# inferrna/Core

Hardware: AMD Instinct MI355X
Metric: Mrays/s (primary+shadow), 1M-tri scene (higher is better)
Workload: dtype f32

## Files before the change

core_amd/csrc/yk_device.hip:

```cpp
#include <hip/hip_runtime.h>

#include <algorithm>
#include <atomic>
#include <climits>
#include <chrono>
#include <cmath>
#include <cstdio>
#include <cstdlib>
#include <cstring>
#include <mutex>
#include <type_traits>
#include <stdexcept>
#include <string>
#include <thread>
#include <vector>

#include "../../include/yk_api.h"
#include "../../include/yk_test_hooks.h"
#include "../../include/yk_test_hooks_light.h"
#include "../../include/yk_test_hooks_camera.h"
#include "../../include/yk_test_hooks_film.h"
#include "../../include/yk_test_hooks_depth.h"
#include "photon_map.h"
#include "scene.h"
// ... 788 lines not shown
  std::conditional_t<CLOSEST, unsigned long long, unsigned> keys[YK_SMALL_LANE_LEAF ? 1 : 64];
  float s_tmin[(CLOSEST || UNI) ? 64 : 1];
  unsigned ray_n0[64];
  unsigned res_slot[CLOSEST ? 1 : 128];
  float4 cand[CLOSEST ? 64 : 1];
  uint2 stack[R * 64];
};
__host__ __device__ __forceinline__ unsigned small_rec_word(unsigned nn) { return (nn * 6u + 3u) & ~3u; }
__device__ __forceinline__ void small_scene_copy(const DScene& S, uint32_t* dst, int W) {
  const unsigned nthr = 64u * (unsigned)W;
  const unsigned n4 = S.nnodes * 4u, n6 = S.nnodes * 6u;
  for (unsigned i = threadIdx.x; i < n6; i += nthr) {
    const unsigned node = i < n4 ? i >> 2 : (i - n4) >> 1, w = i < n4 ? i & 3u : 4u + ((i - n4) & 1u);
    dst[i] = S.pk[node * kPkWords + w];
  }
  float* t = reinterpret_cast<float*>(dst + small_rec_word(S.nnodes));
  const unsigned nt = S.ntris * 12u, nl = S.nlref * 12u;
  for (unsigned i = threadIdx.x; i < nt + nl; i += nthr) {
    const bool own = i < nt;
    const unsigned j = own ? i : i - nt, rec = j / 12u, w = j - rec * 12u, c = w & 3u;
    const float* src = own ? S.tris : S.ltris;
    t[i] = c < 3u ? src[rec * kTriWords + (w >> 2) * 3u + c] : 0.f;
  }
}
size_t small_scene_bytes(size_t nn, size_t ntris, size_t nlref) {
  return 4 * (((6 * nn + 3) & ~(size_t)3) + 12 * (ntris + nlref));
}

constexpr unsigned kTmaxInf = 0xFFC00000u;
__device__ __forceinline__ float shadow_w(float tmax) {
  return tmax < 0.f ? __uint_as_float(kTmaxInf) : (tmax != tmax ? __uint_as_float(0x7FC00000u) : fabsf(tmax));
}
__device__ __forceinline__ yk_ray unpack_shadow(float4 dw, float4 o) {
  yk_ray r;
  r.from[0] = o.x;
  r.from[1] = o.y;
  r.from[2] = o.z;
  r.dir[0] = dw.x;
  r.dir[1] = dw.y;
  r.dir[2] = dw.z;
  const bool inf = __float_as_uint(dw.w) == kTmaxInf, mis = !inf && (__float_as_uint(dw.w) >> 31) != 0u;
  r.tmin = mis ? YK_MIN_RAYDIST : o.w;
  r.tmax = inf ? -1.f : (mis ? -dw.w : dw.w);
  return r;
}

struct RaySrc {
  const yk_ray* rays;
  const float4* sdir;
  const float4* sorg;
  unsigned omask, kshift, kstride;
};

template <bool CLOSEST, int NSEG, bool TS = false, bool BIG = false, bool UNI = false, int W = 1, bool SPLIT = false>
__device__ __forceinline__ void trace_body(DScene S, RaySrc src, const unsigned* __restrict__ idx,
                                           RayCount rc, yk_hit* __restrict__ hits, uint8_t* __restrict__ occl,
                                           unsigned long long* __restrict__ work, unsigned long long* __restrict__ ctr,
                                           uint2* __restrict__ ovf, int ovf_depth, int refill_min,
                                           float* __restrict__ tsf = nullptr, int ts_depth = 0) {
  using KeyT = std::conditional_t<CLOSEST, unsigned long long, unsigned>;
  constexpr int R = W > 1 ? YK_SMALL_RING : (CLOSEST ? kStackLdsC : kStackLds);
  unsigned* otab;
  uint2* lds;
  float* s_tmin;
  unsigned* res_slot;
  unsigned* ray_n0;
  KeyT* keys;
  float4* cand;
  const char* nbase;
  const char* nbase2 = nullptr;
  const float *tb, *lb;
  unsigned wv = 0;
  int lane;
  if constexpr (W == 1) {
    __shared__ unsigned a_otab[64];
    __shared__ uint2 a_lds[R * 64];
    __shared__ float a_tmin[(CLOSEST || UNI) ? 64 : 1];
    __shared__ unsigned a_res[(!CLOSEST && !TS) ? 128 : 1];
    __shared__ unsigned a_n0[64];
    __shared__ KeyT a_keys[64];
    __shared__ float4 a_cand[CLOSEST ? 64 : 1];
    otab = a_otab;
    lds = a_lds;
    s_tmin = a_tmin;
    res_slot = a_res;
    ray_n0 = a_n0;
    keys = a_keys;
    cand = a_cand;
    nbase = reinterpret_cast<const char*>(S.pk);
    tb = S.tris;
    lb = S.ltris;
    lane = threadIdx.x;
  } else {
    __shared__ WaveLds<CLOSEST, UNI, R> s_w[W];
    wv = (unsigned)__builtin_amdgcn_readfirstlane((int)threadIdx.x) >> 6;
    WaveLds<CLOSEST, UNI, R>& L = s_w[wv];
    otab = L.otab;
    lds = L.stack;
    s_tmin = L.s_tmin;
    res_slot = L.res_slot;
    ray_n0 = L.ray_n0;
    keys = L.keys;
    cand = L.cand;
    uint32_t* dst = reinterpret_cast<uint32_t*>(yk_dyn_lds);
    small_scene_copy(S, dst, W);
    __syncthreads();
    nbase = reinterpret_cast<const char*>(dst);
    nbase2 = reinterpret_cast<const char*>(dst + S.nnodes * 4u);
    tb = reinterpret_cast<const float*>(dst + small_rec_word(S.nnodes));
    lb = tb + S.ntris * 12u;
    lane = threadIdx.x & 63u;
  }
  const unsigned gw = blockIdx.x * (unsigned)W + wv;
  unsigned npend = 0;
  const long long n = __builtin_amdgcn_readfirstlane((int)rc.get());
  if (gw == 0 && lane == 0 && n > 0) atomicAdd(&ctr[3], (unsigned long long)n);
  if ((long long)gw * 64 >= n + 63) return;
  const LaneStackT<R> stk{lds, ovf, (unsigned)ovf_depth, gw};
  int rid = -1;
  bool exhausted = false;
  Trav st;
  unsigned nnodes = 0, ntris = 0, nerr = 0;
#ifndef YK_POOL_CHUNKS
#define YK_POOL_CHUNKS 16
#endif
#ifndef YK_POOL_CHUNK_MAX
#define YK_POOL_CHUNK_MAX 512
#endif
  const unsigned kPoolChunk = (unsigned)__builtin_amdgcn_readfirstlane((int)max(
      64u, min(min((unsigned)YK_POOL_CHUNK_MAX, S.chunk_max),
               (unsigned)(n / ((long long)gridDim.x * W * YK_POOL_CHUNKS)) & ~63u)));
  unsigned xcc;
  asm volatile("s_getreg_b32 %0, hwreg(HW_REG_XCC_ID, 0, 4)" : "=s"(xcc));
  constexpr unsigned kAll = (1u << NSEG) - 1u;
  const unsigned seg_len = (unsigned)((n + NSEG - 1) / NSEG);
  unsigned pool_next = 0, pool_end = 0;
  unsigned seg_done = 0;

  unsigned iters = 0;
#ifdef YK_TRAV_STATS
  unsigned long long s_it = 0, s_act = 0, s_dmax = 0, s_lmax = 0, s_refill = 0;
  unsigned long long c_ref = 0, c_desc = 0, c_leaf = 0, c_pop = 0, c_t0 = clock64();
#endif
  for (;;) {
    const unsigned long long want = __ballot(rid < 0 && !exhausted);
    const unsigned long long act = __ballot(rid >= 0);
    if (want != 0ull && (act == 0ull || __popcll(want) >= refill_min)) {
#ifdef YK_TRAV_STATS
      s_refill++;
#endif
      const unsigned cnt = (unsigned)__popcll(want);
      const unsigned avail = pool_end - pool_next;
      unsigned cb = 0, ce = 0;
      if (avail < cnt && seg_done != kAll) {
#pragma unroll 1
        for (unsigned k = 0; k < (unsigned)NSEG; ++k) {
          const unsigned sgi = (xcc + k) % (unsigned)NSEG;
          if (seg_done & (1u << sgi)) continue;
          const unsigned long long s0 = (unsigned long long)sgi * seg_len;
          const unsigned long long s1 = min(s0 + seg_len, (unsigned long long)n);
          unsigned long long base = 0;
          if (lane == 0) base = atomicAdd(work + 16 * sgi, (unsigned long long)kPoolChunk);
          base = s0 + shfl_u64(base, 0);
          if (base < s1) {
            cb = (unsigned)__builtin_amdgcn_readfirstlane((int)(unsigned)base);
            ce = (unsigned)__builtin_amdgcn_readfirstlane((int)(unsigned)min(base + kPoolChunk, s1));
            break;
          }
          seg_done |= 1u << sgi;
        }
      }
      if (rid < 0 && !exhausted) {
        const unsigned rank = __builtin_amdgcn_mbcnt_hi((unsigned)(want >> 32),
                                                         __builtin_amdgcn_mbcnt_lo((unsigned)want, 0u));
        long long q = -1;
        if (rank < avail) q = pool_next + rank;
        else if (rank - avail < ce - cb) q = cb + (rank - avail);
        if (q < 0) {
          exhausted = (seg_done == kAll);
        } else {
          int r;
          yk_ray ray;
          if constexpr (!SPLIT) {
            r = idx ? (int)idx[q] : (int)q;
            ray = src.rays[r];
          } else {
            const unsigned e = idx ? idx[q] : (unsigned)q, oi = e & src.omask;
            r = (int)((e >> src.kshift) * src.kstride + oi);
            ray = unpack_shadow(src.sdir[r], src.sorg[oi]);
          }
          if (TS) st.ts_max = ts_depth;
          if (trav_begin<CLOSEST, TS, UNI>(S, st, ray)) {
            rid = r;
            ray_n0[lane_fresh()] = nnodes;
            if (CLOSEST || UNI) s_tmin[lane_fresh()] = st.tmin;
          } else if (CLOSEST) {
#ifndef YK_NO_CLOSEST_RESULTS
            const unsigned m1 = vconst<0xFFFFFFFFu>(), z = vconst<0u>();
            hits[r] = yk_hit{(int)m1, __uint_as_float(z), __uint_as_float(z), __uint_as_float(z)};
#endif
          } else {
            occl[r] = 0;
            if (TS) {
              tsf[3 * (size_t)r] = 1.f;
              tsf[3 * (size_t)r + 1] = 1.f;
              tsf[3 * (size_t)r + 2] = 1.f;
            }
          }
        }
      }
      if (avail < cnt) {
        const unsigned take = min(cnt - avail, ce - cb);
        pool_next = cb + take;
        pool_end = ce;
      } else {
        pool_next += cnt;
      }
      pool_next = (unsigned)__builtin_amdgcn_readfirstlane((int)pool_next);
      pool_end = (unsigned)__builtin_amdgcn_readfirstlane((int)pool_end);
    }
#ifdef YK_TRAV_STATS
    {
      const unsigned long long t = clock64();
      c_ref += t - c_t0;
      c_t0 = t;
    }
#endif
    if (__ballot(rid >= 0) == 0ull) {
      if (__ballot(!exhausted) == 0ull) break;
      continue;
    }
    bool runaway = false;
    if ((++iters & 31u) == 0u) runaway = rid >= 0 && nnodes - ray_n0[lane_fresh()] > S.nnodes + 2u;
#ifdef YK_TRAV_STATS
    const unsigned n_before = nnodes, t_before = ntris;
    s_it++;
    s_act += (unsigned long long)__popcll(__ballot(rid >= 0));
#endif
    if constexpr (!TS) {
      const bool act = rid >= 0;
      bool live = false;
      uint32_t w0 = 0, nref = 0;
      bool paused = false;
      if (act) live = trav_descend<CLOSEST, (W > 1)>(S, nbase, nbase2, st, stk, nnodes, w0, nref, paused);
#ifdef YK_TRAV_STATS
      asm volatile("s_waitcnt vmcnt(0) lgkmcnt(0)" ::: "memory");
      {
        const unsigned long long t = clock64();
        c_desc += t - c_t0;
        c_t0 = t;
      }
#endif
      bool occ = false;
      if constexpr (W > 1 && YK_SMALL_LANE_LEAF)
        lane_leaves<CLOSEST, UNI>(tb, lb, st, (live && !paused) ? nref : 0u, w0, cand, s_tmin, ntris, occ);
      else
        coop_leaves<CLOSEST, BIG, UNI, W>(S, tb, lb, st, (live && !paused) ? nref : 0u, w0, keys, cand, otab, s_tmin,
                                           ntris, occ);
#ifdef YK_TRAV_STATS
      asm volatile("s_waitcnt vmcnt(0) lgkmcnt(0)" ::: "memory");
      {
        const unsigned long long t = clock64();
        c_leaf += t - c_t0;
        c_t0 = t;
      }
#endif
      bool fin = false;
      int fin_rid = 0;
      if (act) {
        bool done = !live || occ || (!paused && trav_next<CLOSEST>(S, st, stk));
        if (runaway) {
          st.sp = kSpError;
          done = true;
        }
        const bool err = st.sp == kSpError;
        if (err) nerr++;
        if (done) {
          if (CLOSEST) {
            yk_hit h{-1, 0.f, 0.f, 0.f};
            if (st.Z < st.dist && !err) {
              const float4 c = cand[lane_fresh()];
              unsigned p = __float_as_uint(c.w);
// ... 93 lines not shown
  if (!CLOSEST && !TS && npend) {
    wave_lds_sync<W>();
    const int l = lane_fresh();
    if ((unsigned)l < npend) {
      const unsigned e = res_slot[l];
#ifndef YK_NO_SHADOW_RESULTS
      occl[e >> 1] = (uint8_t)(e & 1u);
#endif
    }
  }
  unsigned long long a = nnodes, b = ntris;
#pragma unroll
  for (int off = 32; off > 0; off >>= 1) {
    a += shfl_u64(a, lane ^ off);
    b += shfl_u64(b, lane ^ off);
  }
  if (lane == 0 && (a | b)) {
    atomicAdd(&ctr[0], a);
    atomicAdd(&ctr[1], b);
  }
  if (nerr) atomicAdd(&ctr[2], (unsigned long long)nerr);
}

#ifndef YK_SHADOW_SEGS
#define YK_SHADOW_SEGS 8
#endif
#ifndef YK_CLOSEST_WAVES
#define YK_CLOSEST_WAVES 7
#endif
#ifndef YK_SHADOW_WAVES
#define YK_SHADOW_WAVES 7
#endif

__global__ void __launch_bounds__(64) __attribute__((amdgpu_waves_per_eu(YK_CLOSEST_WAVES)))
k_trace_closest(DScene S, RaySrc src, const unsigned* __restrict__ idx, RayCount n,
                yk_hit* __restrict__ hits, uint8_t* __restrict__ occl, unsigned long long* __restrict__ work,
                unsigned long long* __restrict__ ctr, uint2* __restrict__ ovf, int ovf_depth, int refill_min) {
  trace_body<true, 8>(S, src, idx, n, hits, occl, work, ctr, ovf, ovf_depth, refill_min);
}
__global__ void __launch_bounds__(64) __attribute__((amdgpu_waves_per_eu(YK_SHADOW_WAVES)))
k_trace_shadow(DScene S, RaySrc src, const unsigned* __restrict__ idx, RayCount n,
               yk_hit* __restrict__ hits, uint8_t* __restrict__ occl, unsigned long long* __restrict__ work,
               unsigned long long* __restrict__ ctr, uint2* __restrict__ ovf, int ovf_depth, int refill_min) {
  trace_body<false, YK_SHADOW_SEGS>(S, src, idx, n, hits, occl, work, ctr, ovf, ovf_depth, refill_min);
}
__global__ void __launch_bounds__(64) __attribute__((amdgpu_waves_per_eu(YK_SHADOW_WAVES)))
k_trace_shadow_split(DScene S, RaySrc src, const unsigned* __restrict__ idx, RayCount n,
                     yk_hit* __restrict__ hits, uint8_t* __restrict__ occl, unsigned long long* __restrict__ work,
                     unsigned long long* __restrict__ ctr, uint2* __restrict__ ovf, int ovf_depth, int refill_min) {
  trace_body<false, YK_SHADOW_SEGS, false, false, false, 1, true>(S, src, idx, n, hits, occl, work, ctr, ovf,
                                                                   ovf_depth, refill_min);
}
__global__ void __launch_bounds__(64) __attribute__((amdgpu_waves_per_eu(YK_CLOSEST_WAVES)))
k_trace_closest_big(DScene S, RaySrc src, const unsigned* __restrict__ idx, RayCount n,
                    yk_hit* __restrict__ hits, uint8_t* __restrict__ occl, unsigned long long* __restrict__ work,
                    unsigned long long* __restrict__ ctr, uint2* __restrict__ ovf, int ovf_depth, int refill_min) {
  trace_body<true, 8, false, true>(S, src, idx, n, hits, occl, work, ctr, ovf, ovf_depth, refill_min);
}
__global__ void __launch_bounds__(64) __attribute__((amdgpu_waves_per_eu(YK_SHADOW_WAVES)))
k_trace_shadow_big(DScene S, RaySrc src, const unsigned* __restrict__ idx, RayCount n,
                   yk_hit* __restrict__ hits, uint8_t* __restrict__ occl, unsigned long long* __restrict__ work,
                   unsigned long long* __restrict__ ctr, uint2* __restrict__ ovf, int ovf_depth, int refill_min) {
  trace_body<false, 1, false, true>(S, src, idx, n, hits, occl, work, ctr, ovf, ovf_depth, refill_min);
}
__global__ void __launch_bounds__(64) __attribute__((amdgpu_waves_per_eu(YK_SHADOW_WAVES)))
k_trace_shadow_uni(DScene S, RaySrc src, const unsigned* __restrict__ idx, RayCount n,
                   yk_hit* __restrict__ hits, uint8_t* __restrict__ occl, unsigned long long* __restrict__ work,
                   unsigned long long* __restrict__ ctr, uint2* __restrict__ ovf, int ovf_depth, int refill_min) {
  trace_body<false, 1, false, false, true>(S, src, idx, n, hits, occl, work, ctr, ovf, ovf_depth,
                                                        refill_min);
}
__global__ void __launch_bounds__(64) __attribute__((amdgpu_waves_per_eu(YK_SHADOW_WAVES)))
k_trace_shadow_big_uni(DScene S, RaySrc src, const unsigned* __restrict__ idx, RayCount n,
                       yk_hit* __restrict__ hits, uint8_t* __restrict__ occl, unsigned long long* __restrict__ work,
                       unsigned long long* __restrict__ ctr, uint2* __restrict__ ovf, int ovf_depth, int refill_min) {
  trace_body<false, 1, false, true, true>(S, src, idx, n, hits, occl, work, ctr, ovf, ovf_depth, refill_min);
}
__global__ void __launch_bounds__(64) __attribute__((amdgpu_waves_per_eu(5)))
k_trace_shadow_ts(DScene S, RaySrc src, const unsigned* __restrict__ idx, RayCount n,
                  uint8_t* __restrict__ occl, float* __restrict__ tsf, int ts_depth, unsigned long long* __restrict__ work,
                  unsigned long long* __restrict__ ctr, uint2* __restrict__ ovf, int ovf_depth, int refill_min) {
  trace_body<false, 1, true>(S, src, idx, n, nullptr, occl, work, ctr, ovf, ovf_depth, refill_min, tsf,
                                    ts_depth);
}
__global__ void __launch_bounds__(64 * YK_SMALL_W) __attribute__((amdgpu_waves_per_eu(YK_CLOSEST_WAVES)))
k_trace_closest_small(DScene S, RaySrc src, const unsigned* __restrict__ idx, RayCount n,
                      yk_hit* __restrict__ hits, uint8_t* __restrict__ occl, unsigned long long* __restrict__ work,
                      unsigned long long* __restrict__ ctr, uint2* __restrict__ ovf, int ovf_depth, int refill_min) {
  trace_body<true, 8, false, false, false, YK_SMALL_W>(S, src, idx, n, hits, occl, work, ctr, ovf, ovf_depth,
                                                       refill_min);
}
__global__ void __launch_bounds__(64 * YK_SMALL_W) __attribute__((amdgpu_waves_per_eu(YK_SHADOW_WAVES)))
k_trace_shadow_small(DScene S, RaySrc src, const unsigned* __restrict__ idx, RayCount n,
                     yk_hit* __restrict__ hits, uint8_t* __restrict__ occl, unsigned long long* __restrict__ work,
                     unsigned long long* __restrict__ ctr, uint2* __restrict__ ovf, int ovf_depth, int refill_min) {
  trace_body<false, YK_SHADOW_SEGS, false, false, false, YK_SMALL_W>(S, src, idx, n, hits, occl, work, ctr, ovf,
                                                                     ovf_depth, refill_min);
}
__global__ void __launch_bounds__(64 * YK_SMALL_W) __attribute__((amdgpu_waves_per_eu(YK_SHADOW_WAVES)))
k_trace_shadow_small_split(DScene S, RaySrc src, const unsigned* __restrict__ idx, RayCount n,
                           yk_hit* __restrict__ hits, uint8_t* __restrict__ occl, unsigned long long* __restrict__ work,
                           unsigned long long* __restrict__ ctr, uint2* __restrict__ ovf, int ovf_depth,
                           int refill_min) {
  trace_body<false, YK_SHADOW_SEGS, false, false, false, YK_SMALL_W, true>(S, src, idx, n, hits, occl, work, ctr,
                                                                           ovf, ovf_depth, refill_min);
}
__global__ void __launch_bounds__(64 * YK_SMALL_W) __attribute__((amdgpu_waves_per_eu(YK_SHADOW_WAVES)))
k_trace_shadow_uni_small(DScene S, RaySrc src, const unsigned* __restrict__ idx, RayCount n,
                         yk_hit* __restrict__ hits, uint8_t* __restrict__ occl, unsigned long long* __restrict__ work,
                         unsigned long long* __restrict__ ctr, uint2* __restrict__ ovf, int ovf_depth, int refill_min) {
  trace_body<false, 1, false, false, true, YK_SMALL_W>(S, src, idx, n, hits, occl, work, ctr, ovf, ovf_depth,
                                                       refill_min);
}



__device__ __forceinline__ SurfPt make_surface(const DScene& S, v3 from, v3 dir, const yk_hit& h) {
  SurfPt sp;
  sp.P = vadd(from, vmul(h.t, dir));
  const float4 g = S.ng[h.prim];
  sp.Ng = V3(g.x, g.y, g.z);
  sp.N = sp.Ng;
  const int mw = __float_as_int(g.w);
  sp.mat = mw & (kSmoothBit - 1);
  if (mw & kSmoothBit) {
    const float* vn = S.vn + 9 * (size_t)h.prim;
    const float b0 = S.uni ? 0.0f : 1.0f - (h.b1 + h.b2);
    sp.N = vnormalize(vadd(vadd(vmul(b0, ld3(vn)), vmul(h.b1, ld3(vn + 3))), vmul(h.b2, ld3(vn + 6))));
  }
  create_cs(sp.N, sp.NU, sp.NV);
  return sp;
}

__device__ __forceinline__ v3 face_forward(v3 Ng, v3 N, v3 I) {
  return (vdot(Ng, I) < 0.f) ? vneg(N) : N;
}

__device__ __forceinline__ float mat_fresnel(const DMat& M, v3 wo, v3 N) {
  if (!M.fresnel) return 1.f;
  const float c = fabsf(N.x * wo.x + N.y * wo.y + N.z * wo.z);
  const float t = M.ior2 + c * c;
  const float g = (t < 1.f) ? 0.f : sqrtf(t - 1.f);
  const float gc = g + c, aux = gc * c;
// ... 2348 lines not shown
  return (v >= 1 && v <= kPipes) ? v : kPipes;
}

constexpr long long kNodeBytes = 116;
const char* plan_batches(const yk_batch_plan_in& in, yk_batch_plan& out) {
  out = yk_batch_plan{};
  out.status = YK_ERR_UNSUPPORTED;
  if (in.slots > (1 << 20) || in.bounces < 0 || in.bounces > 62) return "too many shadow slots or bounces";
  const int K = std::max(1, in.slots);
  const int pipes_cfg = std::min(kPipes, std::max(1, in.pipes));
  const long long owned = std::max<long long>(0, in.owned_tiles);
  const int regions = in.merged ? in.bounces + 1 : 1;
  out.regions = regions;
  const long long region_bytes = in.split ? 34ll * K + 16 : 50ll * K;
  const long long bytes_per_sample = 400 + 2ll * K + region_bytes + (long long)(regions - 1) * (region_bytes + 32) +
                                     (in.transp_shadows ? 28ll * K : 0) + ((in.reserved & 1) ? 4 : 0);
  out.bytes_per_sample = bytes_per_sample;
  const long long target_env = in.target_samples > 0 ? in.target_samples : (32ll << 20);
  const long long target =
      std::min(target_env, std::max(1ll << 20, std::max<long long>(0, in.budget_bytes) / pipes_cfg / bytes_per_sample));
  const long long tile_samples = (long long)in.tile * in.tile * in.spp;
  if (in.tile < 1 || in.spp < 1) return "empty tile";
  const long long spec_worst = (2ll << std::max(0, std::min(in.spec_levels, 19))) - 1;
  if (in.spec && spec_worst * tile_samples * kNodeBytes > (48ll << 30))
    return "raydepth too large for the tile size / spp (node store > 48 GB)";
  const long long target_spec = in.spec ? std::min(target, (12ll << 30) / (kNodeBytes * spec_worst)) : target;
  const long long tiles_fill = in.spec ? LLONG_MAX : (owned + pipes_cfg - 1) / pipes_cfg;
  long long tiles_per_batch =
      std::max<long long>(1, std::min<long long>(INT_MAX, std::min(target_spec / tile_samples, tiles_fill)));
  auto index_fits = [&](long long mc) {
    if (mc >= (1ll << 31)) return false;
    int kshift = 0;
    while ((1ll << kshift) < mc * regions) ++kshift;
    return mc * (long long)K * regions < (1ll << 31) && kshift <= 31 && ((long long)(K - 1) << kshift) < (1ll << 32);
  };
  while (tiles_per_batch > 1 && !index_fits(tiles_per_batch * tile_samples)) tiles_per_batch /= 2;
  const long long maxc = tiles_per_batch * tile_samples;
  if (!index_fits(maxc)) return "one tile holds too many samples (tile^2 * spp * shadow slots * regions >= 2^31)";
  out.tiles_per_batch = (int)tiles_per_batch;
  out.maxc = maxc;
  out.kstride = maxc * regions;
  while ((1ll << out.kshift) < out.kstride) ++out.kshift;
  out.nbatch = (int)((owned + tiles_per_batch - 1) / tiles_per_batch);
  out.npipes = in.spec ? 1 : std::min(pipes_cfg, std::max(1, out.nbatch));
  out.status = YK_OK;
  return nullptr;
}

enum TraceVariant {
  kClosest, kShadow, kShadowSplit,
  kClosestBig, kShadowBig,
  kShadowUni, kShadowBigUni,
  kClosestSmall, kShadowSmall, kShadowSmallSplit, kShadowUniSmall,
  kTraceVariants
};
using TraceKernel = void (*)(DScene, RaySrc, const unsigned*, RayCount, yk_hit*, uint8_t*, unsigned long long*,
                             unsigned long long*, uint2*, int, int);
struct TraceInfo {
  TraceKernel kernel;
  int waves;
  bool dyn_lds;
  int ring;
};
constexpr TraceInfo kTrace[kTraceVariants] = {
    {k_trace_closest, 1, false, kStackLdsC},
    {k_trace_shadow, 1, false, kStackLds},
    {k_trace_shadow_split, 1, false, kStackLds},
    {k_trace_closest_big, 1, false, kStackLdsC},
    {k_trace_shadow_big, 1, false, kStackLds},
    {k_trace_shadow_uni, 1, false, kStackLds},
    {k_trace_shadow_big_uni, 1, false, kStackLds},
    {k_trace_closest_small, YK_SMALL_W, true, YK_SMALL_RING},
    {k_trace_shadow_small, YK_SMALL_W, true, YK_SMALL_RING},
    {k_trace_shadow_small_split, YK_SMALL_W, true, YK_SMALL_RING},
    {k_trace_shadow_uni_small, YK_SMALL_W, true, YK_SMALL_RING},
};

struct yk_device {
  int ordinal = 0;
  int cus = 0;
  int per_cu[kTraceVariants] = {};
  bool small = false;
  size_t small_bytes = 0;
  hipStream_t stream = nullptr;
  bool uploaded = false;
  const yk_scene* uploaded_scene = nullptr;
  uint64_t uploaded_gen = 0;
  uint64_t const_token = 0;
  size_t nleaf = 0;
  DBuf<float> tris;
  DBuf<float4> ng;
  DBuf<float> vn;
  DBuf<uint2> nodes;
  DBuf<uint32_t> pk;
  DBuf<float> ltris;
  DBuf<uint32_t> leaf;
  DScene S{};
  int ntris = 0, max_depth = 0, nlights = 0, sum_light_slots = 0;
  bool spec = false;
  int xl_lights = 0;
  DBuf<DMeshLight> ml_recs;
  DBuf<float> ml_f;
  DBuf<uint2> ml_nodes;
  DBuf<uint32_t> ml_leaf;
  bool diff_only = false;
  yk_abort_fn abort_fn = nullptr;
  void* abort_user = nullptr;
  bool big_leaves = false;
  bool crowded_leaves = false;
  int refill = 24;
  int refill_shadow = 24;
  int per_cu_ts = 1;
  int per_cu_lookup[2] = {1, 1};
  DBuf<float> nE, nD, nP, nrcol, nalpha, nmalpha;
  DBuf<int> nflags, nchild, noverflow;
  DBuf<yk_ray> nray;
  DBuf<unsigned> nsoffs, npsample;
  DBuf<unsigned long long> ncount, spec_words;
  bool has_bg = false;
  float bg[3] = {0.f, 0.f, 0.f};
  std::vector<DLight> lights_host;
  bool pm_ready = false;
  int pm_integrator = -1;
  yk_photon_params pm_params{};
  DBuf<uint2> dm_nodes, rm_nodes, cm_nodes;
  DBuf<float4> dm_pos, dm_dir, dm_col, rm_pos, rm_dir, rm_col, cm_pos, cm_dir, cm_col;
  DBuf<uint4> rm_pk;
  std::vector<float> dm_host, rm_host, cm_host;
// ... 345 lines not shown
        *err = "kd-tree leaf " + std::to_string(i) + " references out of range";
        return -1;
      }
      continue;
    }
    const uint64_t r = w1 >> 2;
    if (i + 1 >= nn || r <= i + 1 || r >= nn) {
      *err = "kd-tree node " + std::to_string(i) + " has a child out of order or range";
      return -1;
    }
    for (const uint64_t c : {(uint64_t)i + 1, r}) {
      if (++parents[c] > 1) {
        *err = "kd-tree node " + std::to_string(c) + " has two parents";
        return -1;
      }
      if (depth[i] >= kMaxTreeDepth) {
        *err = "kd-tree deeper than 64 levels (KD_MAX_STACK)";
        return -1;
      }
      depth[c] = (uint8_t)(depth[i] + 1);
      maxd = std::max(maxd, (int)depth[c]);
    }
  }
  for (size_t i = 1; i < nn; ++i)
    if (parents[i] != 1) {
      *err = "kd-tree node " + std::to_string(i) + " is unreachable";
      return -1;
    }
  return maxd;
}

void set_tree_bounds(yk_device* d, int depth) {
  d->max_depth = depth;
  d->S.depth_cap = (unsigned)depth + 2u;
}
int stack_depth(const yk_device* d) { return (int)d->S.depth_cap + 2 * (int)kDescTrips + 2; }

int refill_env() {
  static const int v = [] {
    const char* e = std::getenv("YK_REFILL");
    const int r = e ? std::atoi(e) : 0;
    return (r >= 1 && r <= 64) ? r : 0;
  }();
  return v;
}

inline RaySrc ray_src(const yk_ray* r) { return RaySrc{r, nullptr, nullptr, 0u, 0u, 0u}; }
inline RaySrc shadow_src(const Batch& B) {
  if (!B.split) return ray_src(reinterpret_cast<const yk_ray*>(B.s_dir));
  return RaySrc{nullptr, B.s_dir, B.s_dir + (long long)B.K * B.kstride, (1u << B.kshift) - 1u, (unsigned)B.kshift,
                (unsigned)B.kstride};
}

TraceVariant trace_variant(const yk_device* d, bool closest, bool split) {
  const bool small = d->small && !d->big_leaves;
  if (split) return small ? kShadowSmallSplit : kShadowSplit;
  if (small) return closest ? kClosestSmall : d->S.uni ? kShadowUniSmall : kShadowSmall;
  if (closest) return d->big_leaves ? kClosestBig : kClosest;
  if (d->S.uni) return d->big_leaves ? kShadowBigUni : kShadowUni;
  return d->big_leaves ? kShadowBig : kShadow;
}

void fill_trace_occupancy(yk_device* d, bool dyn_lds) {
  for (int v = 0; v < kTraceVariants; ++v) {
    const TraceInfo& t = kTrace[v];
    if (t.dyn_lds != dyn_lds) continue;
    int blocks = 0;
    HIPCHK(hipOccupancyMaxActiveBlocksPerMultiprocessor(&blocks, t.kernel, 64 * t.waves,
                                                        dyn_lds ? d->small_bytes : 0));
    d->per_cu[v] = std::max(1, blocks);
  }
  if (dyn_lds) return;
  d->per_cu[kShadowUni] = d->per_cu[kShadow];
  d->per_cu[kShadowBigUni] = d->per_cu[kShadowBig];
}

template <bool CLOSEST>
void enqueue_trace(yk_device* d, Pipe& P, RaySrc rays, const unsigned* idx, RayCount n, yk_hit* hits,
                   uint8_t* occ, unsigned long long* work, unsigned long long* acc, hipEvent_t ev0, hipEvent_t ev1) {
  const TraceVariant v = trace_variant(d, CLOSEST, !CLOSEST && rays.rays == nullptr);
  const TraceInfo& t = kTrace[v];
  const long long grid = (long long)d->cus * d->per_cu[v];
  const int ovf_depth = std::max(1, stack_depth(d) - t.ring);
  P.ovf.ensure((size_t)ovf_depth * (size_t)grid * 64 * t.waves);
  if (ev0) HIPCHK(hipEventRecord(ev0, P.stream));
  launch(t.kernel, (unsigned)grid, 64 * t.waves, t.dyn_lds ? d->small_bytes : 0, P.stream, d->S, rays, idx, n, hits,
         occ, work, acc, P.ovf.p, ovf_depth, CLOSEST ? d->refill : d->refill_shadow);
  if (ev1) HIPCHK(hipEventRecord(ev1, P.stream));
}

void enqueue_trace_ts(yk_device* d, Pipe& P, RaySrc rays, const unsigned* idx, RayCount n, uint8_t* occ,
                      float* filt, int max_depth, unsigned long long* work, unsigned long long* acc, hipEvent_t ev0,
                      hipEvent_t ev1) {
  const long long grid = (long long)d->cus * d->per_cu_ts;
  const int ovf_depth = std::max(1, stack_depth(d) - kStackLds);
  P.ovf.ensure((size_t)ovf_depth * (size_t)grid * 64);
  if (ev0) HIPCHK(hipEventRecord(ev0, P.stream));
  launch(k_trace_shadow_ts, (unsigned)grid, 64, 0, P.stream, d->S, rays, idx, n, occ, filt, max_depth, work, acc,
         P.ovf.p, ovf_depth, d->refill_shadow);
  if (ev1) HIPCHK(hipEventRecord(ev1, P.stream));
}

bool lookup_lds(const yk_device* d) { return d->rm_depth <= kLdsPStack && d->rm_nnodes < 65536; }
size_t lookup_lds_bytes(int depth) { return (size_t)std::max(1, depth) * 64 * (sizeof(float) + sizeof(unsigned short)); }

inline int ao_slots(const yk_render_params* p) {
  return (p->integrator == YK_INTEGRATOR_DIRECT && p->do_ao) ? std::max(0, p->ao_samples) : 0;
}
bool shadow_split(const yk_device* d, const yk_render_params* p) {
  const char* e = std::getenv("YK_SPLIT");
  const long long K = std::max<long long>(1, (long long)d->sum_light_slots + ao_slots(p));
  return (e ? std::atoi(e) != 0 : K >= 4) && !d->S.uni && !d->big_leaves && !p->transp_shadows;
}

void add_trace_stats(yk_stats* st, bool closest, uint64_t rays, uint64_t nodes, uint64_t tris, double ms,
                     uint64_t launches = 1) {
  if (closest) {
    st->closest_rays += rays;
    st->closest_nodes += nodes;
    st->closest_tris += tris;
    st->ms_closest += ms;
    st->closest_launches += launches;
  } else {
    st->shadow_rays += rays;
    st->shadow_nodes += nodes;
    st->shadow_tris += tris;
    st->ms_shadow += ms;
    st->shadow_launches += launches;
  }
}

template <bool CLOSEST>
void launch_trace(yk_device* d, Pipe& P, const yk_ray* rays, long long n, yk_hit* hits, uint8_t* occ, yk_stats* st,
// ... 514 lines not shown
```

core_amd/csrc/yk_render_host.inc:

```
struct PassSpec {
  int n, off;
  bool multipass;
  const uint8_t* flags;
  float* d_depth = nullptr;
};

namespace {

bool needs_photon_maps(const yk_render_params* p) {
  return p->integrator == YK_INTEGRATOR_PHOTON ||
         (p->integrator == YK_INTEGRATOR_PATH &&
          (p->caustic_type == YK_CAUSTIC_PHOTON || p->caustic_type == YK_CAUSTIC_BOTH)) ||
         (p->integrator == YK_INTEGRATOR_DIRECT && p->dl_caustics != 0);
}

int check_tiles(const yk_render_params* p) {
  const int tile = p->tile_size > 0 ? p->tile_size : 32;
  if (tile > 4096) return set_error(YK_ERR_UNSUPPORTED, "tile_size > 4096");
  const int ntiles = ((p->width + tile - 1) / tile) * ((p->height + tile - 1) / tile);
  if (ntiles >= (1 << 19)) return set_error(YK_ERR_UNSUPPORTED, "too many tiles");
  if (p->tile_order && p->tile_order_len > 0) {
    if (p->tile_order_len != ntiles)
      return set_error(YK_ERR_ARG, "tile_order must list every tile of the render area once");
    std::vector<char> seen((size_t)ntiles, 0);
// ... 98 lines not shown
        for (int yy = Y; yy < Y + H; ++yy)
          for (int xx = X; xx < X + W; ++xx) {
            const size_t px = (size_t)(yy - F.cy0) * F.w + (xx - F.cx0);
            if (!flags[px]) continue;
            L.pmap[px] = (int)nc;
            L.pix.push_back((yy << 16) | xx);
            nc += spp;
          }
      } else {
        nc += (long long)W * H * spp;
      }
      rx0 = std::min(rx0, X);
      ry0 = std::min(ry0, Y);
      rx1 = std::max(rx1, X + W);
      ry1 = std::max(ry1, Y + H);
    }
    L.base[(size_t)bi * (tpb + 1) + (tb1 - tb0)] = (int)nc;
    L.nc_of[bi] = nc;
    L.rect_of[bi] = make_int4(rx0, ry0, rx1, ry1);
  }
}

struct FilmOptions {
  bool clamp, premult;
};
inline FilmOptions film_options(const yk_render_params* p) { return FilmOptions{p->clamp_rgb != 0, p->premult_alpha != 0}; }
void launch_film_gather(hipStream_t stream, const FilmConst& F, const int* pmap, int tb0, int tb1, int4 rect,
                        long long nc, const float4* samples, const float2* sxy, const int* base, char4* pext,
                        float* d_film, FilmOptions opt = FilmOptions{false, false}, const float* depths = nullptr,
                        float* d_depth = nullptr) {
  FilmConst Fb = F;
  Fb.pmap = pmap;
  Fb.tb0 = tb0;
  Fb.tb1 = tb1;
  const int gx0 = std::max(F.cx0, rect.x + F.olo_x), gy0 = std::max(F.cy0, rect.y + F.olo_y);
  const int gx1 = std::min(F.cx1, rect.z + F.ohi_x), gy1 = std::min(F.cy1, rect.w + F.ohi_y);
  const int gw = gx1 - gx0, gh = gy1 - gy0;
  if (nc > 0 && gw > 0 && gh > 0) {
    const long long npix = nc / F.spp;
    launch(k_pixel_extent, grid_for(npix * 64), 256, 0, stream, Fb, sxy, pext, npix);
    auto* gather = opt.clamp ? (opt.premult ? k_film_gather<true, true> : k_film_gather<true, false>)
                             : (opt.premult ? k_film_gather<false, true> : k_film_gather<false, false>);
    if (samples)
      launch(gather, grid_for((long long)gw * gh), 256, 0, stream, Fb, samples, sxy, base, pext, d_film, gx0, gy0, gw,
             gh);
    if (depths)
      launch(k_depth_gather, grid_for((long long)gw * gh), 256, 0, stream, Fb, depths, sxy, base, pext, d_depth, gx0,
             gy0, gw, gh);
  }
}

struct FramePlan : TileLists {
  bool pm, cmap, ao, path, merged, split;
  FilmConst F;
  RenderConst R;
  AOConst AOC;
  PMConst PMC;
  int K;
  int bounces, nsub;
  int spec_levels;
  yk_batch_plan plan;
  int qwords_per_batch, launches_per_batch;
  long long words_per_batch;
};

const char* build_frame_plan(const yk_device* d, const yk_render_params* p, int32_t shard, int32_t nshards,
                             const PassSpec& ps, FramePlan& fp) {
  fp.pm = p->integrator == YK_INTEGRATOR_PHOTON;
  fp.path = p->integrator == YK_INTEGRATOR_PATH;
  const bool pt_cmap = fp.path && (p->caustic_type == YK_CAUSTIC_PHOTON || p->caustic_type == YK_CAUSTIC_BOTH);
  fp.cmap = needs_photon_maps(p) && !fp.pm;
  fp.ao = p->integrator == YK_INTEGRATOR_DIRECT && p->do_ao != 0;
  FilmConst& F = fp.F;
  F = make_film(p);
  F.shard = shard;
  F.nshards = nshards;
  F.spp = ps.n;
  F.d1 = (float)(1.0 / (double)(float)ps.n);
  F.rank_of = nullptr;
  const int spp = F.spp;
  owned_tiles(F, p->tile_order, p->tile_order_len, fp);
  RenderConst& R = fp.R;
  R = RenderConst{};
  R.spp = spp;
  R.nsub = fp.path ? std::max(1, p->path_samples) : 1;
  R.pm_fg = (fp.pm && p->photon.final_gather && !p->photon.show_map) ? 1 : 0;
  R.pm_showmap = (fp.pm && p->photon.show_map) ? 1 : 0;
  if (R.pm_fg) R.nsub = std::max(1, p->photon.fg_samples);
  fp.PMC = needs_photon_maps(p) ? pm_const(d, p->photon) : PMConst{};
  R.bounces = p->bounces;
  R.integrator = p->integrator;
  R.transp_bg = p->transp_background;
  R.nlights = d->nlights;
  R.has_bg = d->has_bg ? 1 : 0;
  for (int k = 0; k < 3; ++k) R.bg[k] = d->bg[k];
  R.d1 = F.d1;
  R.spec = d->spec ? 1 : 0;
  R.trace_caustics =
      (fp.path && (p->caustic_type == YK_CAUSTIC_PATH || p->caustic_type == YK_CAUSTIC_BOTH)) ? 1 : 0;
  R.rdepth = p->raydepth;
  R.level = 0;
  R.multipass = ps.multipass ? 1 : 0;
  R.pass_off = ps.off;
  R.ps = (R.spec || R.multipass) ? 1 : 0;
  fp.K = std::max(1, d->sum_light_slots + ao_slots(p));
  fp.AOC = AOConst{};
  if (fp.ao) {
    fp.AOC.n = p->ao_samples;
    fp.AOC.k0 = d->sum_light_slots;
    fp.AOC.dist = p->ao_distance;
    for (int k = 0; k < 3; ++k) fp.AOC.col[k] = p->ao_color[k];
  }
  fp.spec_levels = d->spec ? std::max(0, std::min(p->raydepth, 19)) : 0;
  const char* merge_env = std::getenv("YK_MERGE");
  fp.merged = !(merge_env && std::atoi(merge_env) == 0) && fp.path && !d->spec && !pt_cmap && !p->transp_shadows &&
              p->path_samples <= 1 && p->bounces >= 1;
  R.merged = fp.merged ? 1 : 0;
  static const long long batch_gb_env = [] {
    const char* e = std::getenv("YK_BATCH_GB");
    const long long v = e ? std::atoll(e) : 0;
    return (v > 0 && v <= 240) ? v : 0ll;
  }();
  fp.split = shadow_split(d, p);
  yk_batch_plan_in pin{};
  pin.slots = fp.K;
  pin.bounces = fp.merged ? p->bounces : 0;
  pin.merged = fp.merged ? 1 : 0;
  pin.split = fp.split ? 1 : 0;
  pin.transp_shadows = p->transp_shadows ? 1 : 0;
  pin.spec = d->spec ? 1 : 0;
  pin.final_gather = R.pm_fg;
  pin.spec_levels = fp.spec_levels;
  pin.tile = F.tile;
  pin.spp = spp;
  pin.pipes = pipes_env();
  pin.reserved = p->z_channel ? 1 : 0;
  pin.owned_tiles = (long long)fp.owned.size();
  const char* target_env = std::getenv("YK_BATCH_SAMPLES");
  pin.target_samples = target_env ? std::atoll(target_env) : 0;
  pin.budget_bytes = (batch_gb_env ? batch_gb_env : (fp.merged ? 192ll : 64ll)) << 30;
  if (const char* why = plan_batches(pin, fp.plan)) return why;
  fp.bounces = fp.path ? R.bounces : (R.pm_fg ? p->photon.fg_bounces + 1 : 0);
  fp.nsub = (fp.path || R.pm_fg) ? R.nsub : 1;
  fp.qwords_per_batch = fp.nsub * (fp.bounces + 1);
  fp.launches_per_batch = 2 + 2 * fp.nsub * fp.bounces + (R.pm_fg ? fp.nsub * fp.bounces : 0);
  fp.words_per_batch = 2ll * fp.qwords_per_batch + 128ll * fp.launches_per_batch;

  build_tile_lists(F, fp.plan.nbatch, fp.plan.tiles_per_batch, spp, ps.flags, fp);
  return nullptr;
}

void upload_frame_plan(yk_device* d, FramePlan& fp) {
  auto up = [](auto& dev, const auto& host, size_t at_least) {
    dev.ensure(std::max(at_least, host.size()));
    if (!host.empty())
      HIPCHK(hipMemcpy(dev.p, host.data(), host.size() * sizeof(host[0]), hipMemcpyHostToDevice));
  };
  up(d->tiles_dev, fp.tiles, 0);
  up(d->base_dev, fp.base, 0);
  if (!fp.pmap.empty()) {
    up(d->pix_dev, fp.pix, 1);
    up(d->pmap_dev, fp.pmap, 0);
  }
  if (!fp.rank_of.empty()) {
    up(d->rank_dev, fp.rank_of, 0);
    fp.F.rank_of = d->rank_dev.p;
  }
}

void bind_pipes(yk_device* d, const yk_render_params* p, const FramePlan& fp, Batch* Bp) {
  const yk_batch_plan& pl = fp.plan;
  for (int pi = 0; pi < pl.npipes; ++pi) {
    Pipe& P = d->pipe[pi];
    const int nb_here = (pl.nbatch - pi + pl.npipes - 1) / pl.npipes;
    P.words.ensure((size_t)(2 * kAccWords + (d->spec ? 0 : fp.words_per_batch * nb_here)));
    HIPCHK(hipMemsetAsync(P.words.p, 0, P.words.n * sizeof(unsigned long long), P.stream));
// ... 9 lines not shown

NodeStore bind_node_store(yk_device* d, const FramePlan& fp) {
  if (!d->spec) return NodeStore{};
  const long long cap = fp.plan.maxc * ((2ll << fp.spec_levels) - 1);
  d->nE.ensure(3 * cap);
  d->nD.ensure(3 * cap);
  d->nP.ensure(3 * cap);
  d->nrcol.ensure(6 * cap);
  d->nalpha.ensure(fp.plan.maxc);
  d->nflags.ensure(cap);
  d->nchild.ensure(2 * cap);
  d->nray.ensure(cap);
  d->nsoffs.ensure(cap);
  d->npsample.ensure(cap);
  d->ncount.ensure(1);
  d->noverflow.ensure(1);
  d->nmalpha.ensure(cap);
  d->spec_words.ensure((size_t)fp.words_per_batch);
  HIPCHK(hipMemsetAsync(d->noverflow.p, 0, sizeof(int), d->pipe[0].stream));
  return NodeStore{d->nE.p,   d->nD.p,     d->nP.p,       d->nflags.p, d->nchild.p,    d->nrcol.p,    d->nalpha.p,
                   d->nray.p, d->nsoffs.p, d->npsample.p, d->ncount.p, (long long)cap, d->noverflow.p, d->nmalpha.p};
}

struct Timed {
  int pipe;
  size_t ev;
  bool closest;
};

bool cam_can_die(const yk_device* d) { return d->cam_host.kind == YK_CAMERA_ANGULAR && d->cam_host.circular != 0; }

struct BatchCtx {
  yk_device* d;
  const yk_render_params* p;
  const FramePlan* fp;
  const PassSpec* ps;
  float* d_film;
  NodeStore NS;
  std::vector<Timed>* timed;
  size_t* evn;
  int pi;
  Pipe* P;
  Batch B;
  unsigned long long* bw;
  int launch;
  unsigned long long* live = nullptr;
  float* zs = nullptr;
  DepthConst DC{};
};

unsigned long long* qw(const BatchCtx& c, int isub, int depth) { return c.bw + isub * (c.fp->bounces + 1) + depth; }
unsigned long long* next_work(BatchCtx& c) { return c.bw + 2ll * c.fp->qwords_per_batch + 128ll * c.launch++; }

void trace(BatchCtx& c, bool closest, RaySrc rays, const unsigned* idx, RayCount n, yk_hit* hits, uint8_t* occ) {
  Pipe& P = *c.P;
  unsigned long long* work = next_work(c);
  const hipEvent_t e0 = P.event(c.evn[c.pi]), e1 = P.event(c.evn[c.pi] + 1);
  c.timed->push_back(Timed{c.pi, c.evn[c.pi], closest});
  c.evn[c.pi] += 2;
  if (closest) enqueue_trace<true>(c.d, P, rays, idx, n, hits, occ, work, P.words.p, e0, e1);
  else if (c.B.ts)
    enqueue_trace_ts(c.d, P, rays, idx, n, occ, c.B.s_filt, c.p->shadow_depth, work, P.words.p + kAccWords, e0, e1);
  else enqueue_trace<false>(c.d, P, rays, idx, n, hits, occ, work, P.words.p + kAccWords, e0, e1);
}
void trace_shadow_slots(BatchCtx& c, const Batch& Bc, RayCount n) {
  trace(c, false, shadow_src(Bc), Bc.s_idx, n, nullptr, Bc.s_occl);
}

void enqueue_photon_mapping(BatchCtx& c, const Batch& Bc, const RenderConst& Rc, long long n) {
  yk_device* d = c.d;
  Pipe& P = *c.P;
  const PMConst& PMC = c.fp->PMC;
  const int fg_bounces = c.p->photon.fg_bounces;
  if (PMC.show_map || !PMC.final_gather) launch(k_pm_post, grid_for(n, 64), 64, 0, P.stream, d->S, Bc, PMC, n);
  for (int isub = 0; isub < (Rc.pm_fg ? c.fp->nsub : 0); ++isub) {
    launch(d->diff_only ? k_fg_start<true> : k_fg_start<false>, grid_for(n, YK_APPEND_BLOCK), YK_APPEND_BLOCK, 0,
           P.stream, d->S, Bc, Rc, n, isub, P.fgl.p, qw(c, isub, 0));
    int qin = 1;
    for (int it = 0; it <= fg_bounces; ++it) {
      const unsigned long long* in_w = qw(c, isub, it);
      unsigned long long* out_w = qw(c, isub, it + 1);
      trace(c, true, ray_src(Bc.q_rays[qin]), nullptr, RayCount{in_w, 32, 0}, Bc.q_hits[qin], nullptr);
      unsigned long long* lk_w = qw(c, isub, it) + c.fp->qwords_per_batch;
      launch(d->diff_only ? k_fg_hit<true> : k_fg_hit<false>, grid_for(n, YK_APPEND_BLOCK), YK_APPEND_BLOCK, 0,
             P.stream, d->S, Bc, Rc, PMC, in_w, it, isub, qin, P.fgl.p, P.fglen.p, out_w, P.lkq.p, lk_w);
      if (it < fg_bounces) trace_shadow_slots(c, Bc, RayCount{out_w, 0, 0});
      const bool lds = lookup_lds(d);
      launch(lds ? k_pm_lookup<true> : k_pm_lookup<false>, (unsigned)((long long)d->cus * d->per_cu_lookup[lds]), 64,
             lds ? lookup_lds_bytes(d->rm_depth) : 0, P.stream, PMC.rmap, PMC.lookup_rad, d->rm_depth, P.lkq.p, lk_w,
             P.fgl.p, next_work(c));
      launch(k_fg_resolve, grid_for(n), 256, 0, P.stream, Bc, Rc, in_w, qin, P.fgl.p);
      qin ^= 1;
    }
  }
  launch(k_pm_finish, grid_for(n, 64), 64, 0, P.stream, d->S, Bc, Rc, PMC, n);
}

void enqueue_post_direct(BatchCtx& c, const Batch& Bc, const RenderConst& Rc, long long n) {
  const FramePlan& fp = *c.fp;
  hipStream_t s = c.P->stream;
  if (fp.pm) enqueue_photon_mapping(c, Bc, Rc, n);
  if (fp.cmap && fp.PMC.cmap.n != 0)
    launch(k_pt_caustic, grid_for(n, 64), 64, 0, s, c.d->S, Bc, fp.PMC, n);
  if (fp.ao) launch(k_resolve_ao, grid_for(n), 256, 0, s, c.d->S, Bc, Rc, fp.AOC, n);
}

void enqueue_entries(BatchCtx& c, const Batch& Bc, const RenderConst& Rc, long long n, long long node_base) {
  yk_device* d = c.d;
  const FramePlan& fp = *c.fp;
  hipStream_t s = c.P->stream;
  const bool merged = fp.merged;
  const bool post_direct_after_bounces = d->spec;
  if (d->spec) {
    HIPCHK(hipMemsetAsync(d->spec_words.p, 0, d->spec_words.n * sizeof(unsigned long long), s));
    c.launch = 0;
  }
  if (c.live && node_base == 0) trace(c, true, ray_src(Bc.p_rays), Bc.s_idx, RayCount{c.live, 0, 0}, Bc.p_hits, nullptr);
  else trace(c, true, ray_src(Bc.p_rays), nullptr, RayCount{nullptr, 0, n}, Bc.p_hits, nullptr);
  if (c.zs && node_base == 0) launch(k_depth_samples, grid_for(n), 256, 0, s, Bc.p_rays, Bc.p_hits, c.zs, c.DC, n);
  launch(shade_primary_fn(d->diff_only, d->xl_lights, fp.ao), grid_for(n, YK_PRIMARY_BLOCK), YK_PRIMARY_BLOCK, 0, s,
         d->S, Bc, Rc, n, qw(c, 0, 0), fp.AOC);
  if (!merged) {
    trace_shadow_slots(c, Bc, RayCount{qw(c, 0, 0), 0, 0});
    launch(k_resolve_primary, grid_for(n), 256, 0, s, Bc, Rc, n);
  }
  if (!post_direct_after_bounces) enqueue_post_direct(c, Bc, Rc, n);
  const int bblock = bounce_block(d->diff_only);
  for (int isub = 0; isub < (fp.path ? fp.nsub : 0); ++isub) {
    if (isub > 0)
      launch(d->diff_only ? k_path_start<true> : k_path_start<false>, grid_for(n, YK_BOUNCE_BLOCK), YK_BOUNCE_BLOCK, 0,
             s, d->S, Bc, Rc, n, isub, qw(c, isub, 0));
    int qin = 1;
    for (int depth = 1; depth <= fp.bounces; ++depth) {
      const unsigned long long* in_w = qw(c, isub, depth - 1);
      unsigned long long* out_w = qw(c, isub, depth);
      trace(c, true, ray_src(Bc.q_rays[qin]), nullptr, RayCount{in_w, 32, 0}, Bc.q_hits[qin], nullptr);
      Batch Bd = Bc;
      if (merged) {
        Bd = merged_region(Bc, depth);
        Bd.mq_words = qw(c, 0, 0);
      }
      launch(shade_bounce_fn(d->diff_only, d->xl_lights), grid_for(n, bblock), bblock, 0, s, d->S, Bd, Rc, in_w, depth,
             isub, qin, out_w);
      if (!merged) {
        trace_shadow_slots(c, Bc, RayCount{out_w, 0, 0});
        launch(k_resolve_bounce, grid_for(n), 256, 0, s, Bc, Rc, in_w, depth, qin);
      }
      qin ^= 1;
    }
  }
  if (post_direct_after_bounces) enqueue_post_direct(c, Bc, Rc, n);
  if (d->spec) {
    launch(k_finish_spec, grid_for(n), 256, 0, s, Bc, Rc, c.NS, node_base, n);
    launch(k_spawn, grid_for(n), 256, 0, s, d->S, Bc, Rc, c.NS, node_base, n);
  } else if (merged) {
    trace_shadow_slots(c, Bc, RayCount{qw(c, 0, 0), 0, 0, fp.plan.regions});
    launch(k_resolve_merged, grid_for(n), 256, 0, s, Bc, Rc, n, fp.bounces);
  } else {
    launch(k_finish, grid_for(n), 256, 0, s, Bc, Rc, n);
  }
}

int enqueue_spec_generations(BatchCtx& c, long long nc) {
  const FramePlan& fp = *c.fp;
  const NodeStore& NS = c.NS;
  hipStream_t s = c.P->stream;
  const long long maxc = fp.plan.maxc;
  const unsigned long long start = (unsigned long long)nc;
  HIPCHK(hipMemcpyAsync(NS.count, &start, sizeof start, hipMemcpyHostToDevice, s));
  enqueue_entries(c, c.B, fp.R, nc, 0);
  long long g0 = 0, g1 = nc;
// ... 456 lines not shown
```

Before: 3504.

## Hand out camera rays to waves in contiguous 64-ray groups

Result: faster. 3593 (median of 6 runs) (+2.5%).

```diff
diff --git a/core_amd/csrc/yk_device.hip b/core_amd/csrc/yk_device.hip
--- a/core_amd/csrc/yk_device.hip
+++ b/core_amd/csrc/yk_device.hip
@@ -864,12 +864,14 @@
   unsigned omask, kshift, kstride;
 };
 
-template <bool CLOSEST, int NSEG, bool TS = false, bool BIG = false, bool UNI = false, int W = 1, bool SPLIT = false>
+template <bool CLOSEST, int NSEG, bool TS = false, bool BIG = false, bool UNI = false, int W = 1, bool SPLIT = false,
+          bool GROUP = false>
 __device__ __forceinline__ void trace_body(DScene S, RaySrc src, const unsigned* __restrict__ idx,
                                            RayCount rc, yk_hit* __restrict__ hits, uint8_t* __restrict__ occl,
                                            unsigned long long* __restrict__ work, unsigned long long* __restrict__ ctr,
                                            uint2* __restrict__ ovf, int ovf_depth, int refill_min,
                                            float* __restrict__ tsf = nullptr, int ts_depth = 0) {
+  static_assert(!GROUP || (CLOSEST && !TS && !UNI && !SPLIT), "the group hand-out serves the camera-ray closest-hit kernels");
   using KeyT = std::conditional_t<CLOSEST, unsigned long long, unsigned>;
   constexpr int R = W > 1 ? YK_SMALL_RING : (CLOSEST ? kStackLdsC : kStackLds);
   unsigned* otab;
@@ -945,9 +947,15 @@
   unsigned xcc;
   asm volatile("s_getreg_b32 %0, hwreg(HW_REG_XCC_ID, 0, 4)" : "=s"(xcc));
   constexpr unsigned kAll = (1u << NSEG) - 1u;
-  const unsigned seg_len = (unsigned)((n + NSEG - 1) / NSEG);
+  const unsigned seg_len = GROUP ? ((unsigned)((n + NSEG - 1) / NSEG) + 63u) & ~63u : (unsigned)((n + NSEG - 1) / NSEG);
   unsigned pool_next = 0, pool_end = 0;
   unsigned seg_done = 0;
+#ifndef YK_CAMERA_T
+#define YK_CAMERA_T 0
+#endif
+  unsigned gbase = 0;
+  unsigned long long pending = 0ull;
+  bool drained = false;
 
   unsigned iters = 0;
 #ifdef YK_TRAV_STATS
@@ -955,7 +963,61 @@
   unsigned long long c_ref = 0, c_desc = 0, c_leaf = 0, c_pop = 0, c_t0 = clock64();
 #endif
   for (;;) {
-    const unsigned long long want = __ballot(rid < 0 && !exhausted);
+    if constexpr (GROUP) {
+      const unsigned long long act = __ballot(rid >= 0);
+      bool fresh = false;
+      if (pending == 0ull && !drained && __popcll(act) <= YK_CAMERA_T) {
+        if (pool_next >= pool_end && seg_done != kAll) {
+#pragma unroll 1
+          for (unsigned k = 0; k < (unsigned)NSEG; ++k) {
+            const unsigned sgi = (xcc + k) % (unsigned)NSEG;
+            if (seg_done & (1u << sgi)) continue;
+            const unsigned long long s0 = (unsigned long long)sgi * seg_len;
+            const unsigned long long s1 = min(s0 + seg_len, (unsigned long long)n);
+            unsigned long long base = 0;
+            if (lane == 0) base = atomicAdd(work + 16 * sgi, (unsigned long long)kPoolChunk);
+            base = s0 + shfl_u64(base, 0);
+            if (base < s1) {
+              pool_next = (unsigned)__builtin_amdgcn_readfirstlane((int)(unsigned)base);
+              pool_end = (unsigned)__builtin_amdgcn_readfirstlane((int)(unsigned)min(base + kPoolChunk, s1));
+              break;
+            }
+            seg_done |= 1u << sgi;
+          }
+        }
+        if (pool_next < pool_end) {
+          const unsigned cnt = min(64u, pool_end - pool_next);
+          gbase = pool_next;
+          pending = ~0ull >> (64u - cnt);
+          pool_next += cnt;
+          fresh = true;
+        } else {
+          drained = true;
+        }
+      }
+      const unsigned long long go = pending & ~act;
+      if (go != 0ull && (fresh || (pending & act) == 0ull)) {
+#ifdef YK_TRAV_STATS
+        s_refill++;
+#endif
+        const unsigned l = (unsigned)lane_fresh();
+        if ((go >> l) & 1ull) {
+          const int r = idx ? (int)idx[gbase + l] : (int)(gbase + l);
+          if (trav_begin<CLOSEST, TS, UNI>(S, st, src.rays[r])) {
+            rid = r;
+            ray_n0[l] = nnodes;
+            s_tmin[l] = st.tmin;
+          } else {
+#ifndef YK_NO_CLOSEST_RESULTS
+            const unsigned m1 = vconst<0xFFFFFFFFu>(), z = vconst<0u>();
+            hits[r] = yk_hit{(int)m1, __uint_as_float(z), __uint_as_float(z), __uint_as_float(z)};
+#endif
+          }
+        }
+        pending &= ~go;
+      }
+    }
+    const unsigned long long want = GROUP ? 0ull : __ballot(rid < 0 && !exhausted);
     const unsigned long long act = __ballot(rid >= 0);
     if (want != 0ull && (act == 0ull || __popcll(want) >= refill_min)) {
 #ifdef YK_TRAV_STATS
@@ -1039,7 +1101,7 @@
     }
 #endif
     if (__ballot(rid >= 0) == 0ull) {
-      if (__ballot(!exhausted) == 0ull) break;
+      if (GROUP ? drained && pending == 0ull : __ballot(!exhausted) == 0ull) break;
       continue;
     }
     bool runaway = false;
@@ -1239,6 +1301,20 @@
                                                                    ovf_depth, refill_min);
 }
 __global__ void __launch_bounds__(64) __attribute__((amdgpu_waves_per_eu(YK_CLOSEST_WAVES)))
+k_trace_camera(DScene S, RaySrc src, const unsigned* __restrict__ idx, RayCount n,
+               yk_hit* __restrict__ hits, uint8_t* __restrict__ occl, unsigned long long* __restrict__ work,
+               unsigned long long* __restrict__ ctr, uint2* __restrict__ ovf, int ovf_depth, int refill_min) {
+  trace_body<true, 8, false, false, false, 1, false, true>(S, src, idx, n, hits, occl, work, ctr, ovf, ovf_depth,
+                                                           refill_min);
+}
+__global__ void __launch_bounds__(64) __attribute__((amdgpu_waves_per_eu(YK_CLOSEST_WAVES)))
+k_trace_camera_big(DScene S, RaySrc src, const unsigned* __restrict__ idx, RayCount n,
+                   yk_hit* __restrict__ hits, uint8_t* __restrict__ occl, unsigned long long* __restrict__ work,
+                   unsigned long long* __restrict__ ctr, uint2* __restrict__ ovf, int ovf_depth, int refill_min) {
+  trace_body<true, 8, false, true, false, 1, false, true>(S, src, idx, n, hits, occl, work, ctr, ovf, ovf_depth,
+                                                          refill_min);
+}
+__global__ void __launch_bounds__(64) __attribute__((amdgpu_waves_per_eu(YK_CLOSEST_WAVES)))
 k_trace_closest_big(DScene S, RaySrc src, const unsigned* __restrict__ idx, RayCount n,
                     yk_hit* __restrict__ hits, uint8_t* __restrict__ occl, unsigned long long* __restrict__ work,
                     unsigned long long* __restrict__ ctr, uint2* __restrict__ ovf, int ovf_depth, int refill_min) {
@@ -1276,6 +1352,13 @@
                       unsigned long long* __restrict__ ctr, uint2* __restrict__ ovf, int ovf_depth, int refill_min) {
   trace_body<true, 8, false, false, false, YK_SMALL_W>(S, src, idx, n, hits, occl, work, ctr, ovf, ovf_depth,
                                                        refill_min);
+}
+__global__ void __launch_bounds__(64 * YK_SMALL_W) __attribute__((amdgpu_waves_per_eu(YK_CLOSEST_WAVES)))
+k_trace_camera_small(DScene S, RaySrc src, const unsigned* __restrict__ idx, RayCount n,
+                     yk_hit* __restrict__ hits, uint8_t* __restrict__ occl, unsigned long long* __restrict__ work,
+                     unsigned long long* __restrict__ ctr, uint2* __restrict__ ovf, int ovf_depth, int refill_min) {
+  trace_body<true, 8, false, false, false, YK_SMALL_W, false, true>(S, src, idx, n, hits, occl, work, ctr, ovf,
+                                                                    ovf_depth, refill_min);
 }
 __global__ void __launch_bounds__(64 * YK_SMALL_W) __attribute__((amdgpu_waves_per_eu(YK_SHADOW_WAVES)))
 k_trace_shadow_small(DScene S, RaySrc src, const unsigned* __restrict__ idx, RayCount n,
@@ -3730,6 +3813,7 @@
   kClosestBig, kShadowBig,
   kShadowUni, kShadowBigUni,
   kClosestSmall, kShadowSmall, kShadowSmallSplit, kShadowUniSmall,
+  kCamera, kCameraBig, kCameraSmall,
   kTraceVariants
 };
 using TraceKernel = void (*)(DScene, RaySrc, const unsigned*, RayCount, yk_hit*, uint8_t*, unsigned long long*,
@@ -3752,6 +3836,9 @@
     {k_trace_shadow_small, YK_SMALL_W, true, YK_SMALL_RING},
     {k_trace_shadow_small_split, YK_SMALL_W, true, YK_SMALL_RING},
     {k_trace_shadow_uni_small, YK_SMALL_W, true, YK_SMALL_RING},
+    {k_trace_camera, 1, false, kStackLdsC},
+    {k_trace_camera_big, 1, false, kStackLdsC},
+    {k_trace_camera_small, YK_SMALL_W, true, YK_SMALL_RING},
 };
 
 struct yk_device {
@@ -4203,8 +4290,14 @@
                 (unsigned)B.kstride};
 }
 
-TraceVariant trace_variant(const yk_device* d, bool closest, bool split) {
+bool camera_groups() {
+  const char* e = std::getenv("YK_CAMERA_GROUPS");
+  return !(e && std::atoi(e) == 0);
+}
+
+TraceVariant trace_variant(const yk_device* d, bool closest, bool split, bool camera = false) {
   const bool small = d->small && !d->big_leaves;
+  if (closest && camera) return small ? kCameraSmall : d->big_leaves ? kCameraBig : kCamera;
   if (split) return small ? kShadowSmallSplit : kShadowSplit;
   if (small) return closest ? kClosestSmall : d->S.uni ? kShadowUniSmall : kShadowSmall;
   if (closest) return d->big_leaves ? kClosestBig : kClosest;
@@ -4228,8 +4321,9 @@
 
 template <bool CLOSEST>
 void enqueue_trace(yk_device* d, Pipe& P, RaySrc rays, const unsigned* idx, RayCount n, yk_hit* hits,
-                   uint8_t* occ, unsigned long long* work, unsigned long long* acc, hipEvent_t ev0, hipEvent_t ev1) {
-  const TraceVariant v = trace_variant(d, CLOSEST, !CLOSEST && rays.rays == nullptr);
+                   uint8_t* occ, unsigned long long* work, unsigned long long* acc, hipEvent_t ev0, hipEvent_t ev1,
+                   bool camera = false) {
+  const TraceVariant v = trace_variant(d, CLOSEST, !CLOSEST && rays.rays == nullptr, camera);
   const TraceInfo& t = kTrace[v];
   const long long grid = (long long)d->cus * d->per_cu[v];
   const int ovf_depth = std::max(1, stack_depth(d) - t.ring);
diff --git a/core_amd/csrc/yk_render_host.inc b/core_amd/csrc/yk_render_host.inc
--- a/core_amd/csrc/yk_render_host.inc
+++ b/core_amd/csrc/yk_render_host.inc
@@ -174,6 +174,7 @@
 
 struct FramePlan : TileLists {
   bool pm, cmap, ao, path, merged, split;
+  bool cam_groups;
   FilmConst F;
   RenderConst R;
   AOConst AOC;
@@ -244,6 +245,7 @@
     return (v > 0 && v <= 240) ? v : 0ll;
   }();
   fp.split = shadow_split(d, p);
+  fp.cam_groups = camera_groups();
   yk_batch_plan_in pin{};
   pin.slots = fp.K;
   pin.bounces = fp.merged ? p->bounces : 0;
@@ -359,13 +361,14 @@
 unsigned long long* qw(const BatchCtx& c, int isub, int depth) { return c.bw + isub * (c.fp->bounces + 1) + depth; }
 unsigned long long* next_work(BatchCtx& c) { return c.bw + 2ll * c.fp->qwords_per_batch + 128ll * c.launch++; }
 
-void trace(BatchCtx& c, bool closest, RaySrc rays, const unsigned* idx, RayCount n, yk_hit* hits, uint8_t* occ) {
+void trace(BatchCtx& c, bool closest, RaySrc rays, const unsigned* idx, RayCount n, yk_hit* hits, uint8_t* occ,
+           bool camera = false) {
   Pipe& P = *c.P;
   unsigned long long* work = next_work(c);
   const hipEvent_t e0 = P.event(c.evn[c.pi]), e1 = P.event(c.evn[c.pi] + 1);
   c.timed->push_back(Timed{c.pi, c.evn[c.pi], closest});
   c.evn[c.pi] += 2;
-  if (closest) enqueue_trace<true>(c.d, P, rays, idx, n, hits, occ, work, P.words.p, e0, e1);
+  if (closest) enqueue_trace<true>(c.d, P, rays, idx, n, hits, occ, work, P.words.p, e0, e1, camera && c.fp->cam_groups);
   else if (c.B.ts)
     enqueue_trace_ts(c.d, P, rays, idx, n, occ, c.B.s_filt, c.p->shadow_depth, work, P.words.p + kAccWords, e0, e1);
   else enqueue_trace<false>(c.d, P, rays, idx, n, hits, occ, work, P.words.p + kAccWords, e0, e1);
@@ -423,7 +426,7 @@
     c.launch = 0;
   }
   if (c.live && node_base == 0) trace(c, true, ray_src(Bc.p_rays), Bc.s_idx, RayCount{c.live, 0, 0}, Bc.p_hits, nullptr);
-  else trace(c, true, ray_src(Bc.p_rays), nullptr, RayCount{nullptr, 0, n}, Bc.p_hits, nullptr);
+  else trace(c, true, ray_src(Bc.p_rays), nullptr, RayCount{nullptr, 0, n}, Bc.p_hits, nullptr, node_base == 0 && Rc.level == 0);
   if (c.zs && node_base == 0) launch(k_depth_samples, grid_for(n), 256, 0, s, Bc.p_rays, Bc.p_hits, c.zs, c.DC, n);
   launch(shade_primary_fn(d->diff_only, d->xl_lights, fp.ao), grid_for(n, YK_PRIMARY_BLOCK), YK_PRIMARY_BLOCK, 0, s,
          d->S, Bc, Rc, n, qw(c, 0, 0), fp.AOC);
```
